# Nicholasli1995/EgoNet

Hardware: AMD Instinct MI355X
Metric: crops/sec (256x256, heatmap+decode+lift) (higher is better)
Workload: dtype f32; 1 GPU; configs[1]: batch=64 256x256 crops/GPU, HRNet-W48 heatmap head forward + soft decode + affine + FC lifter + pose solve; global_batch=64, weights=synthetic (egonet_amd.synth, seeded per key), parallelism=replicas x1, crops sharded by rank, no collective, ranks=1, backend=none, launch_lanes=1

## Files before the change

### egonet_amd/csrc/conv_fc.hip

```cpp
#include "conv_common.h"

__global__ __launch_bounds__(256, 2) void conv_fc_kernel(ConvArgs a) {
  __shared__ f32x4 red[3][64];
  const int tid = threadIdx.x, lane = tid & 63;
  const int wave = __builtin_amdgcn_readfirstlane(tid >> 6);
  const int li = lane & 15, kq = lane >> 4;
  const int ntile = a.Cout >> 4;
  const int n0 = (blockIdx.x % ntile) * 16, m0 = (blockIdx.x / ntile) * 16;
  const int nchunk = a.nchunk;
  const int rows = a.N * a.H * a.W;

  const __amdgpu_buffer_rsrc_t rx = __builtin_amdgcn_make_buffer_rsrc(
      const_cast<float*>(a.x), 0, (unsigned)((size_t)rows * a.cs_in * 4), EGN_RSRC_WORD3);
  const __amdgpu_buffer_rsrc_t rw = __builtin_amdgcn_make_buffer_rsrc(
      const_cast<float*>(a.w), 0, (unsigned)((size_t)nchunk * EGN_CKQ * a.CoutP * 16), EGN_RSRC_WORD3);
  const unsigned xo = (unsigned)(((m0 + li) * a.cs_in + 4 * kq) * 4);
  const unsigned wo = (unsigned)((kq * a.CoutP + n0 + li) * 16);
  const unsigned wchunk = (unsigned)(EGN_CKQ * a.CoutP * 16);

  f32x4 acc = f32x4{0.f, 0.f, 0.f, 0.f};
  int c = wave;
  for (; c + 12 < nchunk; c += 16) {
    f32x4 xa[4], wb[4];
#pragma unroll
    for (int u = 0; u < 4; ++u) {
      xa[u] = egn_buf_load16(rx, xo + (unsigned)(c + 4 * u) * 64u);
      wb[u] = egn_buf_load16(rw, wo + (unsigned)(c + 4 * u) * wchunk);
    }
#pragma unroll
    for (int u = 0; u < 4; ++u)
#pragma unroll
      for (int e = 0; e < 4; ++e) acc = __builtin_amdgcn_mfma_f32_16x16x4f32(xa[u][e], wb[u][e], acc, 0, 0, 0);
  }
  for (; c < nchunk; c += 4) {
    const f32x4 xa = egn_buf_load16(rx, xo + (unsigned)c * 64u);
    const f32x4 wb = egn_buf_load16(rw, wo + (unsigned)c * wchunk);
#pragma unroll
    for (int e = 0; e < 4; ++e) acc = __builtin_amdgcn_mfma_f32_16x16x4f32(xa[e], wb[e], acc, 0, 0, 0);
  }
  if (wave > 0) red[wave - 1][lane] = acc;
  __syncthreads();
  if (wave != 0) return;
  acc = ((acc + red[0][lane]) + red[1][lane]) + red[2][lane];

  const int act = a.act & EGN_ACT_MASK;
  const bool res_after = (a.act & EGN_ACT_RES_AFTER) != 0;
  const int pitch = a.out_nchw ? a.Cout : a.cs_out;
  const float sc = a.scale[n0 + li], sh = a.shift[n0 + li];
#pragma unroll
  for (int r = 0; r < 4; ++r) {
    const int row = m0 + 4 * kq + r;
    if (row >= rows) continue;
    const size_t o = (size_t)row * pitch + n0 + li;
    float v = __builtin_fmaf(acc[r], sc, sh);
    const float rs = a.res ? a.res[o] : 0.f;
    v = res_after ? rs + egn_act(v, act) : egn_act(v + rs, act);
    a.y[o] = v;
  }
}

bool egn_conv_fc_applies(const ConvArgs& a) {
  const bool one = a.H == 1 && a.W == 1;
  return a.KH == 1 && a.KW == 1 && a.stride == 1 && a.pad == 0 && a.Cin % EGN_CK == 0 && a.cs_in >= a.Cin &&
         a.cs_in % 4 == 0 && a.Cout % 16 == 0 && a.CoutP == a.Cout && (a.out_nchw ? one : a.cs_out >= a.Cout) &&
         a.stats == nullptr && (double)a.N * a.H * a.W * a.cs_in * 4.0 < 2147483648.0;
}

int egn_conv_launch_fc(const ConvArgs& a, hipStream_t stream) {
  if (!egn_conv_fc_applies(a)) return EGN_E_BADARG;
  const int grid = (a.Cout / 16) * ((a.N * a.H * a.W + 15) / 16);
  hipLaunchKernelGGL(conv_fc_kernel, dim3(grid), dim3(256), 0, stream, a);
  return (int)hipGetLastError();
}
```

### egonet_amd/csrc/elementwise.hip

```cpp
#include "egn_internal.h"

struct FuseArgs {
  float* y;
  const float* t[4];
  int shift[4];
  int nterms;
  int N, H, W, cs4;
  int relu;
};

__global__ __launch_bounds__(256) void fuse_sum_relu_kernel(FuseArgs a) {
  const size_t total = (size_t)a.N * a.H * a.W * a.cs4;
  for (size_t e = (size_t)blockIdx.x * blockDim.x + threadIdx.x; e < total;
       e += (size_t)gridDim.x * blockDim.x) {
    const int c4 = (int)(e % a.cs4);
    size_t p = e / a.cs4;
    const int x = (int)(p % a.W);
    p /= a.W;
    const int y = (int)(p % a.H);
    const int n = (int)(p / a.H);
    float4 acc;
#pragma unroll
    for (int k = 0; k < 4; ++k) {
      if (k >= a.nterms) break;
      const int s = a.shift[k];
      const int hs = a.H >> s, ws = a.W >> s;
      const size_t idx = (((size_t)n * hs + (y >> s)) * ws + (x >> s)) * a.cs4 + c4;
      const float4 v = reinterpret_cast<const float4*>(a.t[k])[idx];
      if (k == 0) {
        acc = v;
      } else {
        acc.x += v.x; acc.y += v.y; acc.z += v.z; acc.w += v.w;
      }
    }
    if (a.relu) {
      acc.x = fmaxf(acc.x, 0.f); acc.y = fmaxf(acc.y, 0.f);
      acc.z = fmaxf(acc.z, 0.f); acc.w = fmaxf(acc.w, 0.f);
    }
    reinterpret_cast<float4*>(a.y)[e] = acc;
  }
}

static inline int grid_for(size_t work_items, int block) {
  size_t g = (work_items + block - 1) / block;
  if (g > 2048) g = 2048;
  if (g < 1) g = 1;
  return (int)g;
}

extern "C" int egn_fuse_sum_relu_f32(float* y, int N, int H, int W, int C, int cs,
                                     int nterms, const float* const* terms,
                                     const int* shifts, int relu, void* stream) {
  if (nterms < 1 || nterms > 4 || cs % 4 || C > cs) return EGN_E_BADARG;
  FuseArgs a;
  a.y = y;
  for (int k = 0; k < 4; ++k) { a.t[k] = nullptr; a.shift[k] = 0; }
  for (int k = 0; k < nterms; ++k) {
    a.t[k] = terms[k];
    a.shift[k] = shifts[k];
    if (shifts[k] < 0 || (H >> shifts[k]) << shifts[k] != H || (W >> shifts[k]) << shifts[k] != W)
      return EGN_E_BADARG;
  }
  a.nterms = nterms; a.N = N; a.H = H; a.W = W; a.cs4 = cs / 4; a.relu = relu;
  const size_t total = (size_t)N * H * W * a.cs4;
  hipLaunchKernelGGL(fuse_sum_relu_kernel, dim3(grid_for(total, 256)), dim3(256), 0,
                     (hipStream_t)stream, a);
  return (int)hipGetLastError();
}

__global__ __launch_bounds__(256) void nchw_to_nhwc_kernel(const float* __restrict__ x, float* __restrict__ y,
                                                           int N, int C, int H, int W, int cs4) {
  const size_t hw = (size_t)H * W;
  const size_t total = (size_t)N * cs4 * hw;
  for (size_t e = (size_t)blockIdx.x * blockDim.x + threadIdx.x; e < total;
       e += (size_t)gridDim.x * blockDim.x) {
    const size_t p = e % hw;
    const size_t r = e / hw;
    const int c4 = (int)(r % cs4);
    const int n = (int)(r / cs4);
    float v[4];
#pragma unroll
    for (int k = 0; k < 4; ++k) {
      const int c = c4 * 4 + k;
      v[k] = c < C ? x[((size_t)n * C + c) * hw + p] : 0.f;
    }
    reinterpret_cast<float4*>(y)[((size_t)n * hw + p) * cs4 + c4] = make_float4(v[0], v[1], v[2], v[3]);
  }
}

__global__ __launch_bounds__(256) void nhwc_to_nchw_kernel(const float* __restrict__ x, float* __restrict__ y,
                                                           int N, int C, int H, int W, int cs) {
  const size_t hw = (size_t)H * W;
  const size_t total = (size_t)N * C * hw;
  for (size_t e = (size_t)blockIdx.x * blockDim.x + threadIdx.x; e < total;
       e += (size_t)gridDim.x * blockDim.x) {
    const size_t p = e % hw;
    const size_t r = e / hw;
    const int c = (int)(r % C);
// ... 68 lines not shown
```

### egonet_amd/csrc/conv_common.h

```cpp
#pragma once
#include "egn_internal.h"

typedef float f32x4 __attribute__((ext_vector_type(4)));
typedef unsigned int u32x4 __attribute__((ext_vector_type(4)));

constexpr unsigned EGN_OOB = 0xF0000000u;

typedef __attribute__((address_space(3))) void* egn_lds_ptr_t;
__device__ __forceinline__ unsigned egn_lds_addr(const void* p) {
  return (unsigned)(__UINTPTR_TYPE__)(egn_lds_ptr_t) const_cast<void*>(p);
}

constexpr unsigned EGN_RSRC_WORD3 = 0x00020000u;
struct egn_base48 {
  unsigned lo, hi;
  __device__ __forceinline__ egn_base48(const void* p)
      : lo((unsigned)reinterpret_cast<unsigned long long>(p)),
        hi((unsigned)(reinterpret_cast<unsigned long long>(p) >> 32) & 0xffffu) {}
};
__device__ __forceinline__ u32x4 egn_rsrc(egn_base48 p, unsigned bytes) {
  return u32x4{p.lo, p.hi, bytes, EGN_RSRC_WORD3};
}

#define EGN_LDS_DMA16_ISA(SOFF) "s_mov_b32 m0, %0\n\ts_nop 0\n\tbuffer_load_dwordx4 %1, %2, " SOFF " offen lds"
template <bool MEM = false>
__device__ __forceinline__ void egn_lds_dma16(u32x4 r, unsigned lds_addr, unsigned voff, unsigned soff) {
  if constexpr (MEM) asm volatile(EGN_LDS_DMA16_ISA("%3") : : "s"(lds_addr), "v"(voff), "s"(r), "s"(soff) : "m0", "memory");
  else asm volatile(EGN_LDS_DMA16_ISA("%3") : : "s"(lds_addr), "v"(voff), "s"(r), "s"(soff) : "m0");
}
template <bool MEM = false>
__device__ __forceinline__ void egn_lds_dma16(u32x4 r, unsigned lds_addr, unsigned voff) {
  if constexpr (MEM) asm volatile(EGN_LDS_DMA16_ISA("0") : : "s"(lds_addr), "v"(voff), "s"(r) : "m0", "memory");
  else asm volatile(EGN_LDS_DMA16_ISA("0") : : "s"(lds_addr), "v"(voff), "s"(r) : "m0");
}
#undef EGN_LDS_DMA16_ISA

__device__ __forceinline__ unsigned egn_udiv_magic(unsigned x, unsigned magic) { return magic ? __umulhi(x, magic) : x; }

__device__ __forceinline__ float egn_act(float v, int act) {
  switch (act) {
    case EGN_ACT_RELU: return fmaxf(v, 0.0f);
    case EGN_ACT_SIGMOID: return 1.0f / (1.0f + __expf(-v));
    case EGN_ACT_LEAKY: return v > 0.0f ? v : 0.01f * v;
    default: return v;
  }
}

__device__ __forceinline__ f32x4 egn_buf_load16(__amdgpu_buffer_rsrc_t r, unsigned voff) {
  return __builtin_bit_cast(f32x4, __builtin_amdgcn_raw_buffer_load_b128(r, voff, 0, 0));
}
__device__ __forceinline__ void egn_buf_store16(__amdgpu_buffer_rsrc_t r, unsigned voff, f32x4 v) {
  __builtin_amdgcn_raw_buffer_store_b128(__builtin_bit_cast(u32x4, v), r, voff, 0, 0);
}
__device__ __forceinline__ float egn_buf_load4(__amdgpu_buffer_rsrc_t r, unsigned voff, unsigned soff = 0) {
  return __builtin_bit_cast(float, __builtin_amdgcn_raw_buffer_load_b32(r, voff, soff, 0));
}
__device__ __forceinline__ void egn_buf_store4(__amdgpu_buffer_rsrc_t r, unsigned voff, unsigned soff, float v) {
  __builtin_amdgcn_raw_buffer_store_b32(__builtin_bit_cast(unsigned, v), r, voff, soff, 0);
}
__device__ __forceinline__ void egn_buf_store4(__amdgpu_buffer_rsrc_t r, unsigned voff, float v) {
  egn_buf_store4(r, voff, 0u, v);
}

template <int WM, int MT>
__device__ __forceinline__ void conv_epi_pixels(const ConvArgs& a, float4* smem, int tid, int n_base, int oy0,
                                                int ox0) {
  constexpr int TM = WM * MT * 16;
  int* sPix = reinterpret_cast<int*>(smem + a.spix_off);
  if (tid < TM) {
    const int tile_px = a.TH * a.TW;
    const int b = tid / tile_px;
    const int rem = tid - b * tile_px;
    const int y = rem / a.TW;
    const int x = rem - y * a.TW;
    const int n = n_base + b;
    const int oy = oy0 + y;
    const int ox = ox0 + x;
    sPix[tid] = (b < a.TNB && n < a.N && oy < a.Ho && ox < a.Wo) ? (n * a.Ho + oy) * a.Wo + ox : -1;
  }
}

template <int MT, int NT>
// ... 140 lines not shown
```

### egonet_amd/csrc/conv_dma.hip

```cpp
#include <stdlib.h>

#include "conv_common.h"

__device__ __forceinline__ void egn_dma16(u32x4 r, float4* dst, unsigned voff, int soff) {
#ifdef EGN_DMA_VIA_BUILTIN
  const __amdgpu_buffer_rsrc_t rs = __builtin_amdgcn_make_buffer_rsrc(
      reinterpret_cast<void*>(((unsigned long long)(r[1] & 0xffffu) << 32) | r[0]), 0, r[2], r[3]);
  __builtin_amdgcn_raw_ptr_buffer_load_lds(rs, (egn_lds_ptr_t)dst, 16, voff, soff, 0, 0);
  return;
#endif
  egn_lds_dma16(r, egn_lds_addr(dst), voff, (unsigned)soff);
}

template <int WM, int WN, int MT, int NT, int A_IT, int B_IT, int ABL = 0>
__global__ __launch_bounds__(256, 2) void conv_dma_kernel(ConvArgs a) {
  static_assert(WM * WN == 4, "256-thread workgroups");
  constexpr int NTHREADS = 256;
  constexpr int TN = WN * NT * 16;
  constexpr int CKQ = EGN_CKQ;

  extern __shared__ float4 smem[];
  const int a_slots = a.npixp * CKQ;
  const int b_slots = a.tps * CKQ * TN;
  float4* sA = smem;
  float4* sB = smem + 2 * a_slots;

  const int tid = threadIdx.x;
  const int lane = tid & 63;
  const int wave = __builtin_amdgcn_readfirstlane(tid >> 6);
  const int wm = wave / WN;
  const int wn = wave % WN;
  const int li = lane & 15;
  const int kq = lane >> 4;

  const int tile = blockIdx.x;
  const int tx = tile % a.tiles_x;
  const int ty = (tile / a.tiles_x) % a.tiles_y;
  const int tb = tile / (a.tiles_x * a.tiles_y);
  const int n_base = tb * a.TNB;
  const int oy0 = ty * a.TH;
  const int ox0 = tx * a.TW;
  const int n0 = blockIdx.y * TN;
  const int tile_px = a.TH * a.TW;

  constexpr unsigned OOB = 0xF0000000u;
  const u32x4 rx = egn_rsrc(a.x, (size_t)a.N * a.H * a.W * a.cs_in * 4);
  const u32x4 rw = egn_rsrc(a.w, (size_t)a.nchunk * a.taps * CKQ * a.CoutP * 16);

  const int q = tid & 3;
  const int p0 = tid >> 2;
  unsigned aoff[A_IT];
#pragma unroll
  for (int it = 0; it < A_IT; ++it) {
    const int p = p0 + it * 64;
    unsigned off = OOB;
    if (p < a.npix) {
      const int hx = p % a.HW;
      const int r = p / a.HW;
      const int hy = r % a.HH;
      const int b = r / a.HH;
      const int n = n_base + b;
      const int iy = oy0 * a.stride - a.pad + hy;
      const int ix = ox0 * a.stride - a.pad + hx;
      if ((n < a.N) && (iy >= 0) && (iy < a.H) && (ix >= 0) && (ix < a.W))
        off = (unsigned)(((n * a.H + iy) * a.W + ix) * a.cs_in + q * 4) * 4u;
    }
    aoff[it] = off;
  }
#define EGN_BVOFF(IT)                                                   \
  ((n0 + ((tid + (IT)*NTHREADS) % TN)) < a.CoutP                        \
       ? (unsigned)((((tid + (IT)*NTHREADS) / TN) * a.CoutP) + n0 + ((tid + (IT)*NTHREADS) % TN)) * 16u \
       : OOB)

  int pixbase[MT];
#pragma unroll
  for (int mt = 0; mt < MT; ++mt) {
    const int m = (wm * MT + mt) * 16 + li;
    int b = m / tile_px;
    const int rem = m - b * tile_px;
    const int y = rem / a.TW;
    const int x = rem - y * a.TW;
    if (b >= a.TNB) b = 0;
    pixbase[mt] = ((b * a.HH + y * a.stride) * a.HW + x * a.stride) * CKQ + kq;
  }

  f32x4 acc[MT][NT];
#pragma unroll
  for (int mt = 0; mt < MT; ++mt)
#pragma unroll
    for (int nt = 0; nt < NT; ++nt) acc[mt][nt] = f32x4{0.f, 0.f, 0.f, 0.f};

  const int nspc = (a.taps + a.tps - 1) / a.tps;
  const int nstages = a.nchunk * nspc;

  for (int i = tid; i < 2 * a_slots; i += NTHREADS) sA[i] = make_float4(0.f, 0.f, 0.f, 0.f);
  if (!a.out_nchw) conv_epi_pixels<WM, MT>(a, smem, tid, n_base, oy0, ox0);
  __syncthreads();

#define EGN_DMA(S)                                                                                   \
  {                                                                                                  \
    const int c_ = (S) / nspc;                                                                       \
    const int g_ = (S) - c_ * nspc;                                                                  \
    if (g_ == 0) {                                                                                   \
      float4* dst_ = sA + (c_ & 1) * a_slots + wave * 64;                                            \
      const bool cok_ = (c_ * EGN_CK + q * 4) < a.cs_in;                                             \
      _Pragma("unroll") for (int it = 0; it < A_IT; ++it) {                                          \
        if (it * 64 < a.npix) {                                                                      \
          if (aoff[it] != OOB && cok_)                                                               \
            egn_dma16(rx, dst_ + it * NTHREADS, aoff[it], c_ * EGN_CK * 4);                          \
        }                                                                                            \
      }                                                                                              \
    }                                                                                                \
    const int nts_ = min(a.tps, a.taps - g_ * a.tps);                                                \
    const int b_elems_ = nts_ * CKQ * TN;                                                            \
    const int sw_ = (c_ * a.taps + g_ * a.tps) * CKQ * a.CoutP * 16;                                 \
    float4* dstb_ = sB + ((S)&1) * b_slots + wave * 64;                                              \
    _Pragma("unroll") for (int it = 0; it < B_IT; ++it) {                                            \
      if (wave * 64 + it * NTHREADS < b_elems_)                                                      \
        egn_dma16(rw, dstb_ + it * NTHREADS, EGN_BVOFF(it), sw_);                                    \
    }                                                                                                \
  }

#define EGN_LOADF(AF, BF, TT)                                                                        \
  {                                                                                                  \
    const int t_ = t0 + (TT);                                                                        \
    const int ky_ = t_ / a.KW;                                                                       \
    const int kx_ = t_ - ky_ * a.KW;                                                                 \
    const int dslot_ = (ky_ * a.HW + kx_) * CKQ;                                                     \
    _Pragma("unroll") for (int mt = 0; mt < MT; ++mt) AF[mt] = curA[pixbase[mt] + dslot_];           \
    _Pragma("unroll") for (int nt = 0; nt < NT; ++nt)                                                \
        BF[nt] = curB[((TT)*CKQ + kq) * TN + (wn * NT + nt) * 16 + li];                              \
  }

#define EGN_MFMA(AF, BF)                                                                             \
  _Pragma("unroll") for (int mt = 0; mt < MT; ++mt) _Pragma("unroll") for (int nt = 0; nt < NT; ++nt) { \
    acc[mt][nt] = __builtin_amdgcn_mfma_f32_16x16x4f32(AF[mt].x, BF[nt].x, acc[mt][nt], 0, 0, 0);    \
    acc[mt][nt] = __builtin_amdgcn_mfma_f32_16x16x4f32(AF[mt].y, BF[nt].y, acc[mt][nt], 0, 0, 0);    \
    acc[mt][nt] = __builtin_amdgcn_mfma_f32_16x16x4f32(AF[mt].z, BF[nt].z, acc[mt][nt], 0, 0, 0);    \
    acc[mt][nt] = __builtin_amdgcn_mfma_f32_16x16x4f32(AF[mt].w, BF[nt].w, acc[mt][nt], 0, 0, 0);    \
  }

#ifndef EGN_DMA_INTERLEAVE
#define EGN_INTERLEAVE()
#else
#define EGN_INTERLEAVE()                                                             \
  _Pragma("unroll") for (int k_ = 0; k_ < MT * NT * 4; ++k_) {                       \
    __builtin_amdgcn_sched_group_barrier(0x008, 1, 0);                   \
    __builtin_amdgcn_sched_group_barrier(0x106, 1, 0);  \
  }
#endif

#define EGN_COMPUTE(S)                                                  \
  {                                                                     \
    const int c = (S) / nspc;                                           \
    const int g = (S) - c * nspc;                                       \
    const int t0 = g * a.tps;                                           \
    const int nts = min(a.tps, a.taps - t0);                            \
    const float4* curA = sA + (c & 1) * a_slots;                        \
    const float4* curB = sB + ((S)&1) * b_slots;                        \
    float4 afA[MT], bfA[NT], afB[MT], bfB[NT];                          \
    EGN_LOADF(afA, bfA, 0)                                              \
    for (int tt = 0; tt < nts; tt += 2) {                               \
      if constexpr (ABL == 2) {                                         \
        EGN_MFMA(afA, bfA)                                              \
        if (tt + 1 < nts) EGN_MFMA(afA, bfA)                            \
        continue;                                                       \
      }                                                                 \
       \
       \
      EGN_LOADF(afB, bfB, min(tt + 1, nts - 1))                         \
      EGN_MFMA(afA, bfA)                                                \
      EGN_INTERLEAVE()                                                  \
      if (tt + 1 < nts) {                                               \
        EGN_LOADF(afA, bfA, min(tt + 2, nts - 1))                       \
        EGN_MFMA(afB, bfB)                                              \
        EGN_INTERLEAVE()                                                \
      }                                                                 \
    }                                                                   \
  }

  constexpr bool kStage = (ABL != 1 && ABL != 2);
  if constexpr (kStage) EGN_DMA(0)
  for (int s = 0; s + 1 < nstages; ++s) {
    if constexpr (kStage) {
      __builtin_amdgcn_s_waitcnt(0x0070);
      __syncthreads();
      EGN_DMA(s + 1)
    }
    EGN_COMPUTE(s)
  }
  if constexpr (kStage) {
    __builtin_amdgcn_s_waitcnt(0x0070);
    __syncthreads();
  }
  ConvEpiRegs<MT, NT> er;
  const bool nhwc = !a.out_nchw && ABL != 3;
  if (nhwc) conv_epi_prefetch<WM, WN, MT, NT>(a, smem, tid, n0, er);
  EGN_COMPUTE(nstages - 1)

  if constexpr (ABL == 3) {
#pragma unroll
    for (int mt = 0; mt < MT; ++mt)
#pragma unroll
      for (int nt = 0; nt < NT; ++nt) asm volatile("" ::"v"(acc[mt][nt]));
    return;
  }
  if (nhwc)
    conv_epi_finish<WM, WN, MT, NT>(a, acc, smem, tid, n0, er);
  else
    conv_epi_nchw<WM, WN, MT, NT>(a, acc, tid, n_base, oy0, ox0, n0);
}

template <int WM, int WN, int MT, int NT, int ABL>
static int launch_abl(const ConvArgs& a, size_t lds, hipStream_t stream) {
  static bool raised[EGN_MAX_DEVICES];
  EGN_CHECK_HIP(egn_allow_big_lds(&conv_dma_kernel<WM, WN, MT, NT, 8, 8, ABL>, EGN_BIG_LDS_BYTES, raised));
  const int tiles_b = (a.N + a.TNB - 1) / a.TNB;
  dim3 grid(a.tiles_x * a.tiles_y * tiles_b, (a.CoutP + WN * NT * 16 - 1) / (WN * NT * 16));
  hipLaunchKernelGGL((conv_dma_kernel<WM, WN, MT, NT, 8, 8, ABL>), grid, dim3(256), lds, stream, a);
  return (int)hipGetLastError();
}

template <int WM, int WN, int MT, int NT>
static int launch_one(const ConvArgs& a, size_t lds, hipStream_t stream) {
  static bool raised[EGN_MAX_DEVICES];
  EGN_CHECK_HIP(egn_allow_big_lds(&conv_dma_kernel<WM, WN, MT, NT, 8, 8>, EGN_BIG_LDS_BYTES, raised));
  const int tiles_b = (a.N + a.TNB - 1) / a.TNB;
  dim3 grid(a.tiles_x * a.tiles_y * tiles_b, (a.CoutP + WN * NT * 16 - 1) / (WN * NT * 16));
  hipLaunchKernelGGL((conv_dma_kernel<WM, WN, MT, NT, 8, 8>), grid, dim3(256), lds, stream, a);
  return (int)hipGetLastError();
}

int egn_conv_launch_dma(const ConvArgs& a, DirectTile tile, size_t lds, hipStream_t stream) {
#ifdef EGN_PROBES
  static const int abl = getenv("EGN_CONV_ABLATE") ? atoi(getenv("EGN_CONV_ABLATE")) : 0;
  if (abl && tile == T128x96) {
    if (abl == 1) return launch_abl<2, 2, 4, 3, 1>(a, lds, stream);
    if (abl == 2) return launch_abl<2, 2, 4, 3, 2>(a, lds, stream);
    if (abl == 3) return launch_abl<2, 2, 4, 3, 3>(a, lds, stream);
  }
  if (abl && tile == T128x48) {
    if (abl == 1) return launch_abl<4, 1, 2, 3, 1>(a, lds, stream);
    if (abl == 2) return launch_abl<4, 1, 2, 3, 2>(a, lds, stream);
    if (abl == 3) return launch_abl<4, 1, 2, 3, 3>(a, lds, stream);
  }
#endif
  switch (tile) {
    case T256x48: return launch_one<4, 1, 4, 3>(a, lds, stream);
    case T128x96: return launch_one<2, 2, 4, 3>(a, lds, stream);
    case T128x64: return launch_one<2, 2, 4, 2>(a, lds, stream);
    case T256x16: return launch_one<4, 1, 4, 1>(a, lds, stream);
    case T256x32: return launch_one<4, 1, 4, 2>(a, lds, stream);
    case T128x48: return launch_one<4, 1, 2, 3>(a, lds, stream);
    case T64x96: return launch_one<2, 2, 2, 3>(a, lds, stream);
    case T64x64: return launch_one<2, 2, 2, 2>(a, lds, stream);
    case T64x64_NWaves: return launch_one<1, 4, 4, 1>(a, lds, stream);
    case T32x192: return launch_one<1, 4, 2, 3>(a, lds, stream);
  }
  return EGN_E_BADARG;
}
```

### egonet_amd/csrc/conv_mfma.hip

```cpp
#include "conv_common.h"


template <int WM, int WN, int MT, int NT, int A_IT, int B_IT>
__global__ __launch_bounds__(256, 3) void conv_mfma_kernel(ConvArgs a) {
  static_assert(WM * WN == 4, "256-thread workgroups");
  constexpr int NTHREADS = 256;
  constexpr int TN = WN * NT * 16;
  constexpr int TNW = NT * 16;
  constexpr int TM = WM * MT * 16;
  constexpr int CKQ = EGN_CKQ;

  extern __shared__ float4 smem[];
  float4* sA = smem;
  float4* sB = smem + CKQ * a.npixp;

  const int tid = threadIdx.x;
  const int lane = tid & 63;
  const int wave = tid >> 6;
  const int wm = wave / WN;
  const int wn = wave % WN;
  const int li = lane & 15;
  const int kq = lane >> 4;

  const int tile = blockIdx.x;
  const int tx = tile % a.tiles_x;
  const int ty = (tile / a.tiles_x) % a.tiles_y;
  const int tb = tile / (a.tiles_x * a.tiles_y);
  const int n_base = tb * a.TNB;
  const int oy0 = ty * a.TH;
  const int ox0 = tx * a.TW;
  const int n0 = blockIdx.y * TN;
  const int tile_px = a.TH * a.TW;

  constexpr unsigned OOB = 0xF0000000u;
  const __amdgpu_buffer_rsrc_t rx = __builtin_amdgcn_make_buffer_rsrc(
      const_cast<float*>(a.x), 0, (unsigned)((size_t)a.N * a.H * a.W * a.cs_in * 4), EGN_RSRC_WORD3);
  const __amdgpu_buffer_rsrc_t rw = __builtin_amdgcn_make_buffer_rsrc(
      const_cast<float*>(a.w), 0, (unsigned)((size_t)a.nchunk * a.taps * CKQ * a.CoutP * 16), EGN_RSRC_WORD3);
  const int q = tid & 3;
  const int p0 = tid >> 2;
  unsigned aoff[A_IT];
#pragma unroll
  for (int it = 0; it < A_IT; ++it) {
    const int p = p0 + it * 64;
    unsigned off = OOB;
    if (p < a.npix) {
      const int hx = p % a.HW;
      const int r = p / a.HW;
      const int hy = r % a.HH;
      const int b = r / a.HH;
      const int n = n_base + b;
      const int iy = oy0 * a.stride - a.pad + hy;
      const int ix = ox0 * a.stride - a.pad + hx;
      if ((n < a.N) && (iy >= 0) && (iy < a.H) && (ix >= 0) && (ix < a.W))
        off = (unsigned)(((n * a.H + iy) * a.W + ix) * a.cs_in + q * 4) * 4u;
    }
    aoff[it] = off;
  }
#define EGN_BVOFF(IT)                                                   \
  ((n0 + ((tid + (IT)*NTHREADS) % TN)) < a.CoutP                        \
       ? (unsigned)((((tid + (IT)*NTHREADS) / TN) * a.CoutP) + n0 + ((tid + (IT)*NTHREADS) % TN)) * 16u \
       : OOB)

  if (!a.out_nchw) conv_epi_pixels<WM, MT>(a, smem, tid, n_base, oy0, ox0);

  int pixbase[MT];
#pragma unroll
  for (int mt = 0; mt < MT; ++mt) {
    const int m = (wm * MT + mt) * 16 + li;
    int b = m / tile_px;
    const int rem = m - b * tile_px;
    const int y = rem / a.TW;
    const int x = rem - y * a.TW;
    if (b >= a.TNB) b = 0;
    pixbase[mt] = (b * a.HH + y * a.stride) * a.HW + x * a.stride;
  }

  f32x4 acc[MT][NT];
#pragma unroll
  for (int mt = 0; mt < MT; ++mt)
#pragma unroll
    for (int nt = 0; nt < NT; ++nt) acc[mt][nt] = f32x4{0.f, 0.f, 0.f, 0.f};

  const int nspc = (a.taps + a.tps - 1) / a.tps;
  const int nstages = a.nchunk * nspc;

  f32x4 ra[A_IT], rb[B_IT];

#define EGN_ISSUE(S)                                                                              \
  {                                                                                               \
    const int c_ = (S) / nspc;                                                                    \
    const int g_ = (S) - c_ * nspc;                                                               \
    if (g_ == 0) {                                                                                \
      const bool cpad_ = (c_ * EGN_CK + q * 4) >= a.cs_in;                                        \
      _Pragma("unroll") for (int it = 0; it < A_IT; ++it) ra[it] = __builtin_bit_cast(            \
          f32x4, __builtin_amdgcn_raw_buffer_load_b128(rx, cpad_ ? OOB : aoff[it], c_ * EGN_CK * 4, 0)); \
    }                                                                                             \
    const int sw_ = (c_ * a.taps + g_ * a.tps) * CKQ * a.CoutP * 16;                              \
    _Pragma("unroll") for (int it = 0; it < B_IT; ++it) rb[it] =                                  \
        __builtin_bit_cast(f32x4, __builtin_amdgcn_raw_buffer_load_b128(rw, EGN_BVOFF(it), sw_, 0)); \
  }

  EGN_ISSUE(0)
  for (int s = 0; s < nstages; ++s) {
    __syncthreads();
    {
      const int c = s / nspc;
      const int g = s - c * nspc;
      const int nts = min(a.tps, a.taps - g * a.tps);
      if (g == 0) {
#pragma unroll
        for (int it = 0; it < A_IT; ++it) {
          const int p = p0 + it * 64;
          if (p < a.npix) *reinterpret_cast<f32x4*>(&sA[q * a.npixp + (p ^ (q << 1))]) = ra[it];
        }
      }
      const int b_elems = nts * CKQ * TN;
#pragma unroll
      for (int it = 0; it < B_IT; ++it) {
        const int e = tid + it * NTHREADS;
        if (e < b_elems) *reinterpret_cast<f32x4*>(&sB[e]) = rb[it];
      }
    }
    __syncthreads();
    if (s + 1 < nstages) EGN_ISSUE(s + 1)

    const int g = s % nspc;
    const int t0 = g * a.tps;
    const int nts = min(a.tps, a.taps - t0);
    for (int tt = 0; tt < nts; ++tt) {
      const int t = t0 + tt;
      const int ky = t / a.KW;
      const int kx = t - ky * a.KW;
      const int dpix = ky * a.HW + kx;
      float4 af[MT], bf[NT];
#pragma unroll
      for (int mt = 0; mt < MT; ++mt) af[mt] = sA[kq * a.npixp + ((pixbase[mt] + dpix) ^ (kq << 1))];
#pragma unroll
      for (int nt = 0; nt < NT; ++nt) bf[nt] = sB[(tt * CKQ + kq) * TN + (wn * NT + nt) * 16 + li];
#pragma unroll
      for (int mt = 0; mt < MT; ++mt)
#pragma unroll
        for (int nt = 0; nt < NT; ++nt) {
          acc[mt][nt] = __builtin_amdgcn_mfma_f32_16x16x4f32(af[mt].x, bf[nt].x, acc[mt][nt], 0, 0, 0);
          acc[mt][nt] = __builtin_amdgcn_mfma_f32_16x16x4f32(af[mt].y, bf[nt].y, acc[mt][nt], 0, 0, 0);
          acc[mt][nt] = __builtin_amdgcn_mfma_f32_16x16x4f32(af[mt].z, bf[nt].z, acc[mt][nt], 0, 0, 0);
          acc[mt][nt] = __builtin_amdgcn_mfma_f32_16x16x4f32(af[mt].w, bf[nt].w, acc[mt][nt], 0, 0, 0);
        }
    }
  }

  if (a.out_nchw) {
    conv_epi_nchw<WM, WN, MT, NT>(a, acc, tid, n_base, oy0, ox0, n0);
  } else {
    ConvEpiRegs<MT, NT> er;
    conv_epi_prefetch<WM, WN, MT, NT>(a, smem, tid, n0, er);
    conv_epi_finish<WM, WN, MT, NT>(a, acc, smem, tid, n0, er);
  }
}

template <int WM, int WN, int MT, int NT, int AI, int BI>
static int launch_one(const ConvArgs& a, size_t lds, hipStream_t stream) {
  const int tiles_b = (a.N + a.TNB - 1) / a.TNB;
  dim3 grid(a.tiles_x * a.tiles_y * tiles_b, (a.CoutP + WN * NT * 16 - 1) / (WN * NT * 16));
  hipLaunchKernelGGL((conv_mfma_kernel<WM, WN, MT, NT, AI, BI>), grid, dim3(256), lds, stream, a);
  return (int)hipGetLastError();
}

int egn_conv_launch_staged(const ConvArgs& a, DirectTile tile, size_t lds, hipStream_t stream) {
  switch (tile) {
    case T256x48: return launch_one<4, 1, 4, 3, 6, 7>(a, lds, stream);
    case T128x96: return launch_one<2, 2, 4, 3, 6, 8>(a, lds, stream);
    case T128x64: return launch_one<2, 2, 4, 2, 8, 8>(a, lds, stream);
    case T256x16: return launch_one<4, 1, 4, 1, 8, 8>(a, lds, stream);
    case T256x32: return launch_one<4, 1, 4, 2, 8, 8>(a, lds, stream);
    case T128x48: return launch_one<4, 1, 2, 3, 8, 8>(a, lds, stream);
    case T64x96: return launch_one<2, 2, 2, 3, 8, 8>(a, lds, stream);
    case T64x64: return launch_one<2, 2, 2, 2, 8, 8>(a, lds, stream);
    case T64x64_NWaves: return launch_one<1, 4, 4, 1, 8, 8>(a, lds, stream);
    case T32x192: return launch_one<1, 4, 2, 3, 8, 8>(a, lds, stream);
  }
// ... 3 lines not shown
```

Baseline: 5299 crops/s.

## Add persistent multi-tile 1x1 conv path and run-based upsample-sum fusion

When a 1x1 conv has at least 4096 rows, it now uses a persistent-grid path. Each wave owns a 16-row slab and accumulates up to 6 output tiles, so activation loads are reused across output tiles and the next chunk is prefetched. This replaces the previous split-K scheme, which reduced partial sums across waves through shared memory. Separately, the multi-branch sum+ReLU kernel now processes runs of 4 pixels per thread, reusing each upsampled low-resolution load and switching to 32-bit index math. The new FC path raises register pressure at the higher tile counts, and an environment variable can override the row threshold.

```diff
diff --git a/egonet_amd/csrc/conv_fc.hip b/egonet_amd/csrc/conv_fc.hip
--- a/egonet_amd/csrc/conv_fc.hip
+++ b/egonet_amd/csrc/conv_fc.hip
@@ -1,9 +1,109 @@
+#include <stdlib.h>
 #include "conv_common.h"
+
+#define FC_CHUNK(ACC, XA, WB)                                                                        \
+  _Pragma("unroll") for (int e_ = 0; e_ < 4; ++e_)                                                   \
+      ACC = __builtin_amdgcn_mfma_f32_16x16x4f32((XA)[e_], (WB)[e_], ACC, 0, 0, 0);
+
+template <int NT>
+__device__ __forceinline__ void conv_fc_rows(const ConvArgs& a, int wave, int lane) {
+  const int li = lane & 15, kq = lane >> 4;
+  const int nchunk = a.nchunk, nfull = nchunk & ~3;
+  const int rows = a.N * a.H * a.W;
+  const int ngroup = (a.Cout >> 4) / NT;
+  const int nmb = (rows + 63) >> 6;
+  const int nitem = ((nmb + 7) & ~7) * ngroup;
+
+  const __amdgpu_buffer_rsrc_t rx = __builtin_amdgcn_make_buffer_rsrc(
+      const_cast<float*>(a.x), 0, (unsigned)((size_t)rows * a.cs_in * 4), EGN_RSRC_WORD3);
+  const __amdgpu_buffer_rsrc_t rw = __builtin_amdgcn_make_buffer_rsrc(
+      const_cast<float*>(a.w), 0, (unsigned)((size_t)nchunk * EGN_CKQ * a.CoutP * 16), EGN_RSRC_WORD3);
+  const unsigned wchunk = (unsigned)(EGN_CKQ * a.CoutP * 16);
+  const int act = a.act & EGN_ACT_MASK;
+  const bool res_after = (a.act & EGN_ACT_RES_AFTER) != 0;
+  const int pitch = a.out_nchw ? a.Cout : a.cs_out;
+
+  for (int item = blockIdx.x; item < nitem; item += gridDim.x) {
+    const int q = item >> 3, g = q % ngroup;
+    const int mb = (q / ngroup) * 8 + (item & 7);
+    if (mb >= nmb) continue;
+    const int m0 = (mb * 4 + wave) * 16, n0 = g * NT * 16;
+    if (m0 >= rows) continue;
+    const unsigned xo = (unsigned)(((m0 + li) * a.cs_in + 4 * kq) * 4);
+    const unsigned wo = (unsigned)((kq * a.CoutP + n0 + li) * 16);
+
+    f32x4 acc[NT][4];
+#pragma unroll
+    for (int t = 0; t < NT; ++t)
+#pragma unroll
+      for (int p = 0; p < 4; ++p) acc[t][p] = f32x4{0.f, 0.f, 0.f, 0.f};
+
+    f32x4 xa[4], xn[4] = {}, xt[3];
+#pragma unroll
+    for (int p = 0; p < 3; ++p)
+      xt[p] = nfull + p < nchunk ? egn_buf_load16(rx, xo + (unsigned)(nfull + p) * 64u) : f32x4{0.f, 0.f, 0.f, 0.f};
+    if (nfull > 0) {
+#pragma unroll
+      for (int p = 0; p < 4; ++p) xa[p] = egn_buf_load16(rx, xo + (unsigned)p * 64u);
+    }
+    for (int c = 0; c < nfull; c += 4) {
+      if (c + 4 < nfull) {
+#pragma unroll
+        for (int p = 0; p < 4; ++p) xn[p] = egn_buf_load16(rx, xo + (unsigned)(c + 4 + p) * 64u);
+      }
+#pragma unroll
+      for (int t = 0; t < NT; ++t) {
+        f32x4 wb[4];
+#pragma unroll
+        for (int p = 0; p < 4; ++p) wb[p] = egn_buf_load16(rw, wo + (unsigned)(c + p) * wchunk + (unsigned)t * 256u);
+#pragma unroll
+        for (int p = 0; p < 4; ++p) { FC_CHUNK(acc[t][p], xa[p], wb[p]) }
+      }
+#pragma unroll
+      for (int p = 0; p < 4; ++p) xa[p] = xn[p];
+    }
+#pragma unroll
+    for (int p = 0; p < 3; ++p) {
+      if (nfull + p >= nchunk) break;
+#pragma unroll
+      for (int t = 0; t < NT; ++t) {
+        const f32x4 wb = egn_buf_load16(rw, wo + (unsigned)(nfull + p) * wchunk + (unsigned)t * 256u);
+        FC_CHUNK(acc[t][p], xt[p], wb)
+      }
+    }
+
+#pragma unroll
+    for (int t = 0; t < NT; ++t) {
+      const f32x4 s = ((acc[t][0] + acc[t][1]) + acc[t][2]) + acc[t][3];
+      const int co = n0 + 16 * t + li;
+      const float sc = a.scale[co], sh = a.shift[co];
+#pragma unroll
+      for (int r = 0; r < 4; ++r) {
+        const int row = m0 + 4 * kq + r;
+        if (row >= rows) continue;
+        const size_t o = (size_t)row * pitch + co;
+        float v = __builtin_fmaf(s[r], sc, sh);
+        const float rs = a.res ? a.res[o] : 0.f;
+        v = res_after ? rs + egn_act(v, act) : egn_act(v + rs, act);
+        a.y[o] = v;
+      }
+    }
+  }
+}
 
 __global__ __launch_bounds__(256, 2) void conv_fc_kernel(ConvArgs a) {
   __shared__ f32x4 red[3][64];
   const int tid = threadIdx.x, lane = tid & 63;
   const int wave = __builtin_amdgcn_readfirstlane(tid >> 6);
+  if (a.tps > 0) {
+    switch (a.tps) {
+      case 6: conv_fc_rows<6>(a, wave, lane); break;
+      case 3: conv_fc_rows<3>(a, wave, lane); break;
+      case 2: conv_fc_rows<2>(a, wave, lane); break;
+      default: conv_fc_rows<1>(a, wave, lane); break;
+    }
+    return;
+  }
   const int li = lane & 15, kq = lane >> 4;
   const int ntile = a.Cout >> 4;
   const int n0 = (blockIdx.x % ntile) * 16, m0 = (blockIdx.x / ntile) * 16;
@@ -66,9 +166,35 @@
          a.stats == nullptr && (double)a.N * a.H * a.W * a.cs_in * 4.0 < 2147483648.0;
 }
 
+constexpr int EGN_FC_ROWS = 4096;
+static bool fc_rows_path(int rows) {
+  static const long forced = [] {
+    const char* s = getenv("EGONET_AMD_FC_ROWS");
+    return s && *s ? strtol(s, nullptr, 10) : -1L;
+  }();
+  if (forced >= 0) return forced > 0 && rows >= forced;
+  return rows >= EGN_FC_ROWS;
+}
+
+static int fc_rows_nt(int rows, int ntile) {
+  const long mtiles = (rows + 15) / 16;
+  for (long want : {8L * egn_device_cus(), 4L * egn_device_cus()})
+    for (int nt : {6, 3, 2})
+      if (ntile % nt == 0 && mtiles * (ntile / nt) >= want) return nt;
+  return 1;
+}
+
 int egn_conv_launch_fc(const ConvArgs& a, hipStream_t stream) {
   if (!egn_conv_fc_applies(a)) return EGN_E_BADARG;
-  const int grid = (a.Cout / 16) * ((a.N * a.H * a.W + 15) / 16);
-  hipLaunchKernelGGL(conv_fc_kernel, dim3(grid), dim3(256), 0, stream, a);
+  const int rows = a.N * a.H * a.W;
+  ConvArgs b = a;
+  b.tps = 0;
+  int grid = (a.Cout / 16) * ((rows + 15) / 16);
+  if (fc_rows_path(rows)) {
+    b.tps = fc_rows_nt(rows, a.Cout / 16);
+    const int nmb8 = ((rows + 63) / 64 + 7) / 8 * 8;
+    grid = egn_persistent_grid(nmb8 * (a.Cout / 16 / b.tps), 8, 2);
+  }
+  hipLaunchKernelGGL(conv_fc_kernel, dim3(grid), dim3(256), 0, stream, b);
   return (int)hipGetLastError();
 }
diff --git a/egonet_amd/csrc/elementwise.hip b/egonet_amd/csrc/elementwise.hip
--- a/egonet_amd/csrc/elementwise.hip
+++ b/egonet_amd/csrc/elementwise.hip
@@ -1,44 +1,69 @@
 #include "egn_internal.h"
+
+constexpr int FUSE_RUN = 4;
 
 struct FuseArgs {
   float* y;
   const float* t[4];
   int shift[4];
   int nterms;
-  int N, H, W, cs4;
+  int NH, H, W, cs4;
+  int nruns;
+  unsigned units;
   int relu;
 };
 
 __global__ __launch_bounds__(256) void fuse_sum_relu_kernel(FuseArgs a) {
-  const size_t total = (size_t)a.N * a.H * a.W * a.cs4;
-  for (size_t e = (size_t)blockIdx.x * blockDim.x + threadIdx.x; e < total;
-       e += (size_t)gridDim.x * blockDim.x) {
-    const int c4 = (int)(e % a.cs4);
-    size_t p = e / a.cs4;
-    const int x = (int)(p % a.W);
-    p /= a.W;
-    const int y = (int)(p % a.H);
-    const int n = (int)(p / a.H);
-    float4 acc;
+  const unsigned cs4 = (unsigned)a.cs4, nruns = (unsigned)a.nruns, W = (unsigned)a.W;
+  for (unsigned u = blockIdx.x * 256u + threadIdx.x; u < a.units; u += gridDim.x * 256u) {
+    const unsigned q = u / cs4, c4 = u - q * cs4;
+    const unsigned row = q / nruns, x0 = (q - row * nruns) * FUSE_RUN;
+    const unsigned n = row / (unsigned)a.H, y0 = row - n * (unsigned)a.H;
+    const int npx = (int)(W - x0 < (unsigned)FUSE_RUN ? W - x0 : (unsigned)FUSE_RUN);
+    float4 v[4][FUSE_RUN];
 #pragma unroll
     for (int k = 0; k < 4; ++k) {
       if (k >= a.nterms) break;
       const int s = a.shift[k];
       const int hs = a.H >> s, ws = a.W >> s;
-      const size_t idx = (((size_t)n * hs + (y >> s)) * ws + (x >> s)) * a.cs4 + c4;
-      const float4 v = reinterpret_cast<const float4*>(a.t[k])[idx];
-      if (k == 0) {
-        acc = v;
+      const float4* t = reinterpret_cast<const float4*>(a.t[k]) + (((n * hs + (y0 >> s)) * ws + (x0 >> s)) * cs4 + c4);
+      if (s == 0) {
+#pragma unroll
+        for (int j = 0; j < FUSE_RUN; ++j) v[k][j] = j < npx ? t[j * cs4] : make_float4(0.f, 0.f, 0.f, 0.f);
+      } else if (s == 1) {
+        const float4 l0 = t[0];
+        const float4 l1 = npx > 2 ? t[cs4] : l0;
+        v[k][0] = l0; v[k][1] = l0; v[k][2] = l1; v[k][3] = l1;
       } else {
-        acc.x += v.x; acc.y += v.y; acc.z += v.z; acc.w += v.w;
+        const float4 l0 = t[0];
+#pragma unroll
+        for (int j = 0; j < FUSE_RUN; ++j) v[k][j] = l0;
       }
     }
-    if (a.relu) {
-      acc.x = fmaxf(acc.x, 0.f); acc.y = fmaxf(acc.y, 0.f);
-      acc.z = fmaxf(acc.z, 0.f); acc.w = fmaxf(acc.w, 0.f);
+    float4* y = reinterpret_cast<float4*>(a.y) + ((row * W + x0) * cs4 + c4);
+#pragma unroll
+    for (int j = 0; j < FUSE_RUN; ++j) {
+      if (j >= npx) break;
+      float4 acc = v[0][j];
+#pragma unroll
+      for (int k = 1; k < 4; ++k) {
+        if (k >= a.nterms) break;
+        acc.x += v[k][j].x; acc.y += v[k][j].y; acc.z += v[k][j].z; acc.w += v[k][j].w;
+      }
+      if (a.relu) {
+        acc.x = fmaxf(acc.x, 0.f); acc.y = fmaxf(acc.y, 0.f);
+        acc.z = fmaxf(acc.z, 0.f); acc.w = fmaxf(acc.w, 0.f);
+      }
+      y[j * cs4] = acc;
     }
-    reinterpret_cast<float4*>(a.y)[e] = acc;
   }
+}
+
+static inline int fuse_grid(unsigned units) {
+  const unsigned blocks = (units + 255u) / 256u, cap = 8u * (unsigned)egn_device_cus();
+  if (blocks <= cap) return blocks < 1u ? 1 : (int)blocks;
+  const unsigned steps = (blocks + cap - 1u) / cap;
+  return (int)((blocks + steps - 1u) / steps);
 }
 
 static inline int grid_for(size_t work_items, int block) {
@@ -61,9 +86,11 @@
     if (shifts[k] < 0 || (H >> shifts[k]) << shifts[k] != H || (W >> shifts[k]) << shifts[k] != W)
       return EGN_E_BADARG;
   }
-  a.nterms = nterms; a.N = N; a.H = H; a.W = W; a.cs4 = cs / 4; a.relu = relu;
-  const size_t total = (size_t)N * H * W * a.cs4;
-  hipLaunchKernelGGL(fuse_sum_relu_kernel, dim3(grid_for(total, 256)), dim3(256), 0,
+  if (N < 0 || H < 0 || W < 0 || (double)N * H * W * cs * 4.0 >= 2147483648.0) return EGN_E_BADARG;
+  a.nterms = nterms; a.NH = N * H; a.H = H; a.W = W; a.cs4 = cs / 4; a.relu = relu;
+  a.nruns = (W + FUSE_RUN - 1) / FUSE_RUN;
+  a.units = (unsigned)a.NH * (unsigned)a.nruns * (unsigned)a.cs4;
+  hipLaunchKernelGGL(fuse_sum_relu_kernel, dim3(fuse_grid(a.units)), dim3(256), 0,
                      (hipStream_t)stream, a);
   return (int)hipGetLastError();
 }
```

Measured after the change: 5307 crops/s (median of 3 runs). About the same (+0.2%).

## Stream conv weights directly from global into registers instead of staging in LDS

Applied to the files above, without the earlier changes.

The MFMA conv kernels (staged and DMA variants) no longer stage weight tiles in LDS. Each lane now loads its B fragments straight from global memory with buffer loads, software-pipelined two taps ahead, with a third register set to handle odd tap counts. This removes the LDS writes and reads for weights and the per-tap-group stage split, so only activations remain staged per channel chunk. The cost is more register pressure and exposed global-load latency, since each wave fetches its own weights with no sharing through LDS. An ablation path for the T64x96 tile is also added.

```diff
diff --git a/egonet_amd/csrc/conv_common.h b/egonet_amd/csrc/conv_common.h
--- a/egonet_amd/csrc/conv_common.h
+++ b/egonet_amd/csrc/conv_common.h
@@ -48,6 +48,9 @@
 
 __device__ __forceinline__ f32x4 egn_buf_load16(__amdgpu_buffer_rsrc_t r, unsigned voff) {
   return __builtin_bit_cast(f32x4, __builtin_amdgcn_raw_buffer_load_b128(r, voff, 0, 0));
+}
+__device__ __forceinline__ f32x4 egn_buf_load16(__amdgpu_buffer_rsrc_t r, unsigned voff, unsigned soff) {
+  return __builtin_bit_cast(f32x4, __builtin_amdgcn_raw_buffer_load_b128(r, voff, soff, 0));
 }
 __device__ __forceinline__ void egn_buf_store16(__amdgpu_buffer_rsrc_t r, unsigned voff, f32x4 v) {
   __builtin_amdgcn_raw_buffer_store_b128(__builtin_bit_cast(u32x4, v), r, voff, 0, 0);
diff --git a/egonet_amd/csrc/conv_dma.hip b/egonet_amd/csrc/conv_dma.hip
--- a/egonet_amd/csrc/conv_dma.hip
+++ b/egonet_amd/csrc/conv_dma.hip
@@ -21,9 +21,7 @@
 
   extern __shared__ float4 smem[];
   const int a_slots = a.npixp * CKQ;
-  const int b_slots = a.tps * CKQ * TN;
   float4* sA = smem;
-  float4* sB = smem + 2 * a_slots;
 
   const int tid = threadIdx.x;
   const int lane = tid & 63;
@@ -45,7 +43,6 @@
 
   constexpr unsigned OOB = 0xF0000000u;
   const u32x4 rx = egn_rsrc(a.x, (size_t)a.N * a.H * a.W * a.cs_in * 4);
-  const u32x4 rw = egn_rsrc(a.w, (size_t)a.nchunk * a.taps * CKQ * a.CoutP * 16);
 
   const int q = tid & 3;
   const int p0 = tid >> 2;
@@ -67,11 +64,6 @@
     }
     aoff[it] = off;
   }
-#define EGN_BVOFF(IT)                                                   \
-  ((n0 + ((tid + (IT)*NTHREADS) % TN)) < a.CoutP                        \
-       ? (unsigned)((((tid + (IT)*NTHREADS) / TN) * a.CoutP) + n0 + ((tid + (IT)*NTHREADS) % TN)) * 16u \
-       : OOB)
-
   int pixbase[MT];
 #pragma unroll
   for (int mt = 0; mt < MT; ++mt) {
@@ -90,46 +82,45 @@
 #pragma unroll
     for (int nt = 0; nt < NT; ++nt) acc[mt][nt] = f32x4{0.f, 0.f, 0.f, 0.f};
 
-  const int nspc = (a.taps + a.tps - 1) / a.tps;
-  const int nstages = a.nchunk * nspc;
+  const __amdgpu_buffer_rsrc_t rwb = __builtin_amdgcn_make_buffer_rsrc(
+      const_cast<float*>(a.w), 0, (unsigned)((size_t)a.nchunk * a.taps * CKQ * a.CoutP * 16), EGN_RSRC_WORD3);
+  unsigned bvoff[NT];
+#pragma unroll
+  for (int nt = 0; nt < NT; ++nt) {
+    const int co = n0 + (wn * NT + nt) * 16 + li;
+    bvoff[nt] = co < a.CoutP ? (unsigned)(kq * a.CoutP + co) * 16u : OOB;
+  }
+  const unsigned bstep = (unsigned)(CKQ * a.CoutP * 16);
+  const int ntaps_all = a.nchunk * a.taps;
 
   for (int i = tid; i < 2 * a_slots; i += NTHREADS) sA[i] = make_float4(0.f, 0.f, 0.f, 0.f);
   if (!a.out_nchw) conv_epi_pixels<WM, MT>(a, smem, tid, n_base, oy0, ox0);
   __syncthreads();
 
-#define EGN_DMA(S)                                                                                   \
+#define EGN_DMA(C)                                                                                   \
   {                                                                                                  \
-    const int c_ = (S) / nspc;                                                                       \
-    const int g_ = (S) - c_ * nspc;                                                                  \
-    if (g_ == 0) {                                                                                   \
-      float4* dst_ = sA + (c_ & 1) * a_slots + wave * 64;                                            \
-      const bool cok_ = (c_ * EGN_CK + q * 4) < a.cs_in;                                             \
-      _Pragma("unroll") for (int it = 0; it < A_IT; ++it) {                                          \
-        if (it * 64 < a.npix) {                                                                      \
-          if (aoff[it] != OOB && cok_)                                                               \
-            egn_dma16(rx, dst_ + it * NTHREADS, aoff[it], c_ * EGN_CK * 4);                          \
-        }                                                                                            \
+    float4* dst_ = sA + ((C)&1) * a_slots + wave * 64;                                               \
+    const bool cok_ = ((C)*EGN_CK + q * 4) < a.cs_in;                                                \
+    _Pragma("unroll") for (int it = 0; it < A_IT; ++it) {                                            \
+      if (it * 64 < a.npix) {                                                                        \
+        if (aoff[it] != OOB && cok_) egn_dma16(rx, dst_ + it * NTHREADS, aoff[it], (C)*EGN_CK * 4);  \
       }                                                                                              \
     }                                                                                                \
-    const int nts_ = min(a.tps, a.taps - g_ * a.tps);                                                \
-    const int b_elems_ = nts_ * CKQ * TN;                                                            \
-    const int sw_ = (c_ * a.taps + g_ * a.tps) * CKQ * a.CoutP * 16;                                 \
-    float4* dstb_ = sB + ((S)&1) * b_slots + wave * 64;                                              \
-    _Pragma("unroll") for (int it = 0; it < B_IT; ++it) {                                            \
-      if (wave * 64 + it * NTHREADS < b_elems_)                                                      \
-        egn_dma16(rw, dstb_ + it * NTHREADS, EGN_BVOFF(it), sw_);                                    \
-    }                                                                                                \
-  }
-
-#define EGN_LOADF(AF, BF, TT)                                                                        \
+  }
+
+#define EGN_LOADA(AF, TT)                                                                            \
   {                                                                                                  \
-    const int t_ = t0 + (TT);                                                                        \
+    const int t_ = (TT);                                                                             \
     const int ky_ = t_ / a.KW;                                                                       \
     const int kx_ = t_ - ky_ * a.KW;                                                                 \
     const int dslot_ = (ky_ * a.HW + kx_) * CKQ;                                                     \
     _Pragma("unroll") for (int mt = 0; mt < MT; ++mt) AF[mt] = curA[pixbase[mt] + dslot_];           \
-    _Pragma("unroll") for (int nt = 0; nt < NT; ++nt)                                                \
-        BF[nt] = curB[((TT)*CKQ + kq) * TN + (wn * NT + nt) * 16 + li];                              \
+  }
+
+#define EGN_LOADB(BF, V)                                                                             \
+  {                                                                                                  \
+    const unsigned sw_ = (unsigned)min((V), ntaps_all - 1) * bstep;                                  \
+    _Pragma("unroll") for (int nt = 0; nt < NT; ++nt) BF[nt] = egn_buf_load16(rwb, bvoff[nt], sw_);  \
   }
 
 #define EGN_MFMA(AF, BF)                                                                             \
@@ -150,53 +141,66 @@
   }
 #endif
 
-#define EGN_COMPUTE(S)                                                  \
+#define EGN_COMPUTE(C)                                                  \
   {                                                                     \
-    const int c = (S) / nspc;                                           \
-    const int g = (S) - c * nspc;                                       \
-    const int t0 = g * a.tps;                                           \
-    const int nts = min(a.tps, a.taps - t0);                            \
-    const float4* curA = sA + (c & 1) * a_slots;                        \
-    const float4* curB = sB + ((S)&1) * b_slots;                        \
-    float4 afA[MT], bfA[NT], afB[MT], bfB[NT];                          \
-    EGN_LOADF(afA, bfA, 0)                                              \
-    for (int tt = 0; tt < nts; tt += 2) {                               \
+    const float4* curA = sA + ((C)&1) * a_slots;                        \
+    const int nts = a.taps;                                             \
+    const int u0 = (C)*nts;                                             \
+    float4 afA[MT], afB[MT];                                            \
+    EGN_LOADA(afA, 0)                                                   \
+    int tt = 0;                                                         \
+    for (; tt + 1 < nts; tt += 2) {                                     \
       if constexpr (ABL == 2) {                                         \
         EGN_MFMA(afA, bfA)                                              \
-        if (tt + 1 < nts) EGN_MFMA(afA, bfA)                            \
+        EGN_MFMA(afA, bfA)                                              \
         continue;                                                       \
       }                                                                 \
-       \
-       \
-      EGN_LOADF(afB, bfB, min(tt + 1, nts - 1))                         \
+      EGN_LOADA(afB, tt + 1)                                            \
       EGN_MFMA(afA, bfA)                                                \
       EGN_INTERLEAVE()                                                  \
-      if (tt + 1 < nts) {                                               \
-        EGN_LOADF(afA, bfA, min(tt + 2, nts - 1))                       \
-        EGN_MFMA(afB, bfB)                                              \
-        EGN_INTERLEAVE()                                                \
+      EGN_LOADB(bfA, u0 + tt + 2)                                       \
+      EGN_LOADA(afA, min(tt + 2, nts - 1))                              \
+      EGN_MFMA(afB, bfB)                                                \
+      EGN_INTERLEAVE()                                                  \
+      EGN_LOADB(bfB, u0 + tt + 3 + (tt + 3 == nts ? 1 : 0))             \
+    }                                                                   \
+    if (tt < nts) {                                                     \
+      if constexpr (ABL != 2) {                                         \
+        EGN_LOADB(bfC, u0 + nts)                                        \
+        __builtin_amdgcn_sched_barrier(0);  \
       }                                                                 \
+      EGN_MFMA(afA, bfA)                                                \
     }                                                                   \
   }
-
+#define EGN_TAKE_B()                                                    \
+  if (a.taps & 1) {                                                     \
+    _Pragma("unroll") for (int nt = 0; nt < NT; ++nt) bfA[nt] = bfC[nt]; \
+  }
+
+  f32x4 bfA[NT], bfB[NT], bfC[NT];
+  EGN_LOADB(bfA, 0)
+  EGN_LOADB(bfB, 1)
+  EGN_LOADB(bfC, 0)
   constexpr bool kStage = (ABL != 1 && ABL != 2);
   if constexpr (kStage) EGN_DMA(0)
-  for (int s = 0; s + 1 < nstages; ++s) {
+  for (int c = 0; c + 1 < a.nchunk; ++c) {
     if constexpr (kStage) {
       __builtin_amdgcn_s_waitcnt(0x0070);
       __syncthreads();
-      EGN_DMA(s + 1)
     }
-    EGN_COMPUTE(s)
+    EGN_TAKE_B()
+    if constexpr (kStage) EGN_DMA(c + 1)
+    EGN_COMPUTE(c)
   }
   if constexpr (kStage) {
     __builtin_amdgcn_s_waitcnt(0x0070);
     __syncthreads();
   }
+  EGN_TAKE_B()
   ConvEpiRegs<MT, NT> er;
   const bool nhwc = !a.out_nchw && ABL != 3;
   if (nhwc) conv_epi_prefetch<WM, WN, MT, NT>(a, smem, tid, n0, er);
-  EGN_COMPUTE(nstages - 1)
+  EGN_COMPUTE(a.nchunk - 1)
 
   if constexpr (ABL == 3) {
 #pragma unroll
@@ -243,6 +247,11 @@
     if (abl == 1) return launch_abl<4, 1, 2, 3, 1>(a, lds, stream);
     if (abl == 2) return launch_abl<4, 1, 2, 3, 2>(a, lds, stream);
     if (abl == 3) return launch_abl<4, 1, 2, 3, 3>(a, lds, stream);
+  }
+  if (abl && tile == T64x96) {
+    if (abl == 1) return launch_abl<2, 2, 2, 3, 1>(a, lds, stream);
+    if (abl == 2) return launch_abl<2, 2, 2, 3, 2>(a, lds, stream);
+    if (abl == 3) return launch_abl<2, 2, 2, 3, 3>(a, lds, stream);
   }
 #endif
   switch (tile) {
diff --git a/egonet_amd/csrc/conv_mfma.hip b/egonet_amd/csrc/conv_mfma.hip
--- a/egonet_amd/csrc/conv_mfma.hip
+++ b/egonet_amd/csrc/conv_mfma.hip
@@ -12,7 +12,6 @@
 
   extern __shared__ float4 smem[];
   float4* sA = smem;
-  float4* sB = smem + CKQ * a.npixp;
 
   const int tid = threadIdx.x;
   const int lane = tid & 63;
@@ -57,10 +56,14 @@
     }
     aoff[it] = off;
   }
-#define EGN_BVOFF(IT)                                                   \
-  ((n0 + ((tid + (IT)*NTHREADS) % TN)) < a.CoutP                        \
-       ? (unsigned)((((tid + (IT)*NTHREADS) / TN) * a.CoutP) + n0 + ((tid + (IT)*NTHREADS) % TN)) * 16u \
-       : OOB)
+  unsigned bvoff[NT];
+#pragma unroll
+  for (int nt = 0; nt < NT; ++nt) {
+    const int co = n0 + (wn * NT + nt) * 16 + li;
+    bvoff[nt] = co < a.CoutP ? (unsigned)(kq * a.CoutP + co) * 16u : OOB;
+  }
+  const unsigned bstep = (unsigned)(CKQ * a.CoutP * 16);
+  const int ntaps_all = a.nchunk * a.taps;
 
   if (!a.out_nchw) conv_epi_pixels<WM, MT>(a, smem, tid, n_base, oy0, ox0);
 
@@ -82,71 +85,70 @@
 #pragma unroll
     for (int nt = 0; nt < NT; ++nt) acc[mt][nt] = f32x4{0.f, 0.f, 0.f, 0.f};
 
-  const int nspc = (a.taps + a.tps - 1) / a.tps;
-  const int nstages = a.nchunk * nspc;
+  f32x4 ra[A_IT];
 
-  f32x4 ra[A_IT], rb[B_IT];
-
-#define EGN_ISSUE(S)                                                                              \
+#define EGN_ISSUE(C)                                                                              \
   {                                                                                               \
-    const int c_ = (S) / nspc;                                                                    \
-    const int g_ = (S) - c_ * nspc;                                                               \
-    if (g_ == 0) {                                                                                \
-      const bool cpad_ = (c_ * EGN_CK + q * 4) >= a.cs_in;                                        \
-      _Pragma("unroll") for (int it = 0; it < A_IT; ++it) ra[it] = __builtin_bit_cast(            \
-          f32x4, __builtin_amdgcn_raw_buffer_load_b128(rx, cpad_ ? OOB : aoff[it], c_ * EGN_CK * 4, 0)); \
-    }                                                                                             \
-    const int sw_ = (c_ * a.taps + g_ * a.tps) * CKQ * a.CoutP * 16;                              \
-    _Pragma("unroll") for (int it = 0; it < B_IT; ++it) rb[it] =                                  \
-        __builtin_bit_cast(f32x4, __builtin_amdgcn_raw_buffer_load_b128(rw, EGN_BVOFF(it), sw_, 0)); \
+    const bool cpad_ = ((C)*EGN_CK + q * 4) >= a.cs_in;                                           \
+    _Pragma("unroll") for (int it = 0; it < A_IT; ++it) ra[it] = __builtin_bit_cast(              \
+        f32x4, __builtin_amdgcn_raw_buffer_load_b128(rx, cpad_ ? OOB : aoff[it], (C)*EGN_CK * 4, 0)); \
+  }
+#define EGN_LOADB(BF, V)                                                                             \
+  {                                                                                                  \
+    const unsigned sw_ = (unsigned)min((V), ntaps_all - 1) * bstep;                                  \
+    _Pragma("unroll") for (int nt = 0; nt < NT; ++nt) BF[nt] = egn_buf_load16(rw, bvoff[nt], sw_);   \
+  }
+#define EGN_LOADA(AF, T)                                                                             \
+  {                                                                                                  \
+    const int ky_ = (T) / a.KW;                                                                      \
+    const int dpix_ = ky_ * a.HW + ((T)-ky_ * a.KW);                                                 \
+    _Pragma("unroll") for (int mt = 0; mt < MT; ++mt)                                                \
+        AF[mt] = sA[kq * a.npixp + ((pixbase[mt] + dpix_) ^ (kq << 1))];                             \
+  }
+#define EGN_MFMA(AF, BF)                                                                             \
+  _Pragma("unroll") for (int mt = 0; mt < MT; ++mt) _Pragma("unroll") for (int nt = 0; nt < NT; ++nt) { \
+    acc[mt][nt] = __builtin_amdgcn_mfma_f32_16x16x4f32(AF[mt].x, BF[nt].x, acc[mt][nt], 0, 0, 0);    \
+    acc[mt][nt] = __builtin_amdgcn_mfma_f32_16x16x4f32(AF[mt].y, BF[nt].y, acc[mt][nt], 0, 0, 0);    \
+    acc[mt][nt] = __builtin_amdgcn_mfma_f32_16x16x4f32(AF[mt].z, BF[nt].z, acc[mt][nt], 0, 0, 0);    \
+    acc[mt][nt] = __builtin_amdgcn_mfma_f32_16x16x4f32(AF[mt].w, BF[nt].w, acc[mt][nt], 0, 0, 0);    \
   }
 
+  f32x4 bfA[NT], bfB[NT], bfC[NT];
+  EGN_LOADB(bfA, 0)
+  EGN_LOADB(bfB, 1)
+  EGN_LOADB(bfC, 0)
   EGN_ISSUE(0)
-  for (int s = 0; s < nstages; ++s) {
+  const int nts = a.taps;
+  for (int c = 0; c < a.nchunk; ++c) {
     __syncthreads();
-    {
-      const int c = s / nspc;
-      const int g = s - c * nspc;
-      const int nts = min(a.tps, a.taps - g * a.tps);
-      if (g == 0) {
 #pragma unroll
-        for (int it = 0; it < A_IT; ++it) {
-          const int p = p0 + it * 64;
-          if (p < a.npix) *reinterpret_cast<f32x4*>(&sA[q * a.npixp + (p ^ (q << 1))]) = ra[it];
-        }
-      }
-      const int b_elems = nts * CKQ * TN;
-#pragma unroll
-      for (int it = 0; it < B_IT; ++it) {
-        const int e = tid + it * NTHREADS;
-        if (e < b_elems) *reinterpret_cast<f32x4*>(&sB[e]) = rb[it];
-      }
+    for (int it = 0; it < A_IT; ++it) {
+      const int p = p0 + it * 64;
+      if (p < a.npix) *reinterpret_cast<f32x4*>(&sA[q * a.npixp + (p ^ (q << 1))]) = ra[it];
     }
     __syncthreads();
-    if (s + 1 < nstages) EGN_ISSUE(s + 1)
+    if (nts & 1) {
+#pragma unroll
+      for (int nt = 0; nt < NT; ++nt) bfA[nt] = bfC[nt];
+    }
+    if (c + 1 < a.nchunk) EGN_ISSUE(c + 1)
 
-    const int g = s % nspc;
-    const int t0 = g * a.tps;
-    const int nts = min(a.tps, a.taps - t0);
-    for (int tt = 0; tt < nts; ++tt) {
-      const int t = t0 + tt;
-      const int ky = t / a.KW;
-      const int kx = t - ky * a.KW;
-      const int dpix = ky * a.HW + kx;
-      float4 af[MT], bf[NT];
-#pragma unroll
-      for (int mt = 0; mt < MT; ++mt) af[mt] = sA[kq * a.npixp + ((pixbase[mt] + dpix) ^ (kq << 1))];
-#pragma unroll
-      for (int nt = 0; nt < NT; ++nt) bf[nt] = sB[(tt * CKQ + kq) * TN + (wn * NT + nt) * 16 + li];
-#pragma unroll
-      for (int mt = 0; mt < MT; ++mt)
-#pragma unroll
-        for (int nt = 0; nt < NT; ++nt) {
-          acc[mt][nt] = __builtin_amdgcn_mfma_f32_16x16x4f32(af[mt].x, bf[nt].x, acc[mt][nt], 0, 0, 0);
-          acc[mt][nt] = __builtin_amdgcn_mfma_f32_16x16x4f32(af[mt].y, bf[nt].y, acc[mt][nt], 0, 0, 0);
-          acc[mt][nt] = __builtin_amdgcn_mfma_f32_16x16x4f32(af[mt].z, bf[nt].z, acc[mt][nt], 0, 0, 0);
-          acc[mt][nt] = __builtin_amdgcn_mfma_f32_16x16x4f32(af[mt].w, bf[nt].w, acc[mt][nt], 0, 0, 0);
-        }
+    const int u0 = c * nts;
+    float4 afA[MT], afB[MT];
+    int tt = 0;
+    for (; tt + 1 < nts; tt += 2) {
+      EGN_LOADA(afA, tt)
+      EGN_LOADA(afB, tt + 1)
+      EGN_MFMA(afA, bfA)
+      EGN_LOADB(bfA, u0 + tt + 2)
+      EGN_MFMA(afB, bfB)
+      EGN_LOADB(bfB, u0 + tt + 3 + (tt + 3 == nts ? 1 : 0))
+    }
+    if (tt < nts) {
+      EGN_LOADB(bfC, u0 + nts)
+      __builtin_amdgcn_sched_barrier(0);
+      EGN_LOADA(afA, tt)
+      EGN_MFMA(afA, bfA)
     }
   }
 
```

Result: no change. 5312 crops/s before, 5351 crops/s after (median of 6 runs) (+0.7%).
